# RoboticExplorationLab/TortoiseSat.jl

Measured on AMD Instinct MI355X. Metric: AL-iLQR trajectory solves/sec (1000 knots), higher is better.
Workload: dtype f64

## Files before the change

### tortoisesat.jl_amd/csrc/tsat_device.hpp

```cpp
#pragma once
#include <stdint.h>
#include "../../include/tortoise_hip.h"

#ifdef TSAT_EMU
#include <cmath>
namespace tsat_emu { int lane(); void sync(); void* lds(); double* xch(); }
#define TSAT_DEV inline
#define TSAT_PHASE inline
#define TSAT_FWD inline
#define TSAT_GLOBAL
#define TSAT_CONSTMEM
#define TSAT_LANE() (tsat_emu::lane())
#define TSAT_SYNC() (tsat_emu::sync())
#define TSAT_SYNC_LDS() (tsat_emu::sync())
#define TSAT_SCHED_FENCE() ((void)0)
#define TSAT_WAIT_LDS() ((void)0)
#define TSAT_NO_UNROLL
#define TSAT_ATOMIC_ADD(ptr, v) __atomic_fetch_add((ptr), (v), __ATOMIC_RELAXED)
#define TSAT_ATOMIC_LOAD(ptr) __atomic_load_n((ptr), __ATOMIC_RELAXED)
#define TSAT_UNIFORM_INT(x) (x)
#else
#define TSAT_DEV __device__ __forceinline__
#define TSAT_PHASE __device__ __noinline__
#if defined(TSAT_DENSE)
#define TSAT_FWD __device__ __noinline__
#else
#define TSAT_FWD __device__ __forceinline__
#endif
#if defined(__HIP_DEVICE_COMPILE__) && __HIP_DEVICE_COMPILE__
#define TSAT_GLOBAL __attribute__((address_space(1)))
#define TSAT_CONSTMEM __attribute__((address_space(4)))
#else
#define TSAT_GLOBAL
#define TSAT_CONSTMEM
#endif
#define TSAT_LANE() ((int)threadIdx.x)
#define TSAT_SYNC() __syncthreads()
#define TSAT_SYNC_LDS()                                       \
  do {                                                        \
    __builtin_amdgcn_fence(__ATOMIC_RELEASE, "wavefront");    \
    __builtin_amdgcn_wave_barrier();                          \
    __builtin_amdgcn_fence(__ATOMIC_ACQUIRE, "wavefront");    \
  } while (0)
#define TSAT_SCHED_FENCE() __builtin_amdgcn_sched_barrier(0)
#define TSAT_WAIT_LDS() __builtin_amdgcn_s_waitcnt(0xC07F)
#define TSAT_NO_UNROLL _Pragma("unroll 1")
#define TSAT_ATOMIC_ADD(ptr, v) atomicAdd((ptr), (v))
#define TSAT_ATOMIC_LOAD(ptr) __hip_atomic_load((ptr), __ATOMIC_RELAXED, __HIP_MEMORY_SCOPE_AGENT)
#define TSAT_UNIFORM_INT(x) __builtin_amdgcn_readfirstlane((int)(x))
#endif

#if !defined(TSAT_EMU)
#pragma clang fp contract(on)
#endif

namespace tsat {

#ifdef TSAT_F32
typedef float cfg_real;
#else
typedef double cfg_real;
#endif
typedef double acc_t;
constexpr int RPU = 16 / (int)sizeof(cfg_real);
#ifdef TSAT_JAC32
typedef float jac_t;
#else
typedef cfg_real jac_t;
#endif
constexpr int RPUJ = 16 / (int)sizeof(jac_t);

#if defined(TSAT_F32) && !defined(TSAT_OCC)
#define TSAT_OCC 2
#endif

constexpr int WAVE = 64;
#if defined(TSAT_F32) && TSAT_OCC == 4
constexpr int CK = 16;
#else
constexpr int CK = 32;
#endif
constexpr int PSTRIDE = 64;
constexpr int NSTORE = 12;
constexpr int N_FEW = 4;
enum { P_X0 = 0, P_XF = 7, P_QD = 14, P_QFD = 21, P_RD = 28, P_ULO = 31, P_UHI = 34, P_J = 37, P_JI = 46,
       P_TAU0 = 55, P_DTAU = 56, P_DT = 57,
       P_TAU0L = 61, P_DTAUL = 62 };
constexpr int FS = 7;
template <int ES> struct PkRec {
  static constexpr int FSR = ES ? 6 : FS;
  static constexpr int QQ = 54;
  static constexpr int LX = ES ? 60 : 70, LU = ES ? 66 : 77, LUU = ES ? 69 : 80;
  static constexpr int RECS = ES ? 72 : 84;
  static constexpr int SLOT = (64 / 16) * RECS + RPUJ;
};
struct TvRec {
  static constexpr int FSR = FS, LX = 70, LU = 77, LUU = 80, QQ = 83, RECS = 89;
};
constexpr int TV_CHB = 52;
template <int ES> struct BwdCfg {
  static constexpr int NH = ES ? 6 : 7;
  static constexpr int RECS = PkRec<ES>::RECS;
#if defined(TSAT_F32)
  static constexpr int CHB = (TSAT_OCC == 2) ? (ES ? 63 : 54) : (TSAT_OCC == 3) ? (ES ? 39 : 34) : (ES ? 27 : 23);
#elif defined(TSAT_JAC32) && defined(TSAT_DENSE)
  static constexpr int CHB = ES ? 59 : 50;
#elif defined(TSAT_JAC32)
  static constexpr int CHB = 64;
#elif defined(TSAT_DENSE)
  static constexpr int CHB = ES ? 29 : 25;
#else
  static constexpr int CHB = ES ? 64 : 55;
#endif
};
constexpr int KDW = 24, XUW = 10, LMW = 6, BSW = 9;
template <typename real> constexpr size_t pad16(size_t n) { return (n + (16 / sizeof(real)) - 1) / (16 / sizeof(real)) * (16 / sizeof(real)); }
template <typename real> constexpr size_t xu_stride(int NS) { return pad16<real>((size_t)NS * XUW); }
template <typename real> constexpr size_t kd_stride(int NS) { return (size_t)(NS - 1) * KDW; }
template <typename real> constexpr size_t lam_stride(int NS) { return pad16<real>((size_t)(NS - 1) * LMW); }
template <typename real> constexpr size_t u0_stride(int NS) { return (size_t)(NS - 1) * 3; }

template <typename real>
struct KArgs {
  int T, N, n_tab, max_ls;
  tsat_options opt;
  const real* P;
  const real* BT;
  const int* bidx;
  const int* nk;
  const real* U0;
  real* XU;
  real* KD;
  real* LAM;
  real* CAND;
  tsat_stats* stats;
  double* trace;
  int trace_rows;
  real* JW;
  int pk_few = 0;
  int suspend_at = 0;
  int* live = nullptr;
  int* susp_n = nullptr;
  int* susp_ids = nullptr;
  void* susp_state = nullptr;
};

constexpr int TSAT_JW_REALS_PER_4 = 16 * (4 * 84 + 4);

template <typename real>
struct TPtrs {
  TSAT_GLOBAL real* XU;
  TSAT_GLOBAL real* KD;
  TSAT_GLOBAL real* LAM;
  TSAT_GLOBAL real* CAND;
  const TSAT_GLOBAL real* bt;
  TSAT_GLOBAL real* XU0;
  int cur;
};
TSAT_DEV int cand_slab(int cur, int c) { return (c < cur) ? c : c + 1; }
template <typename real>
TSAT_DEV TSAT_GLOBAL real* slab_ptr(const TPtrs<real>& p, int N, int id) {
  return (id == 0) ? p.XU0 : p.CAND + (size_t)(id - 1) * (size_t)N * XUW;
}

constexpr int L_RED = 0;
constexpr int L_TR = L_RED + 64;
constexpr int TR_HJI = PSTRIDE, TR_HH = PSTRIDE + 9, TR_US = PSTRIDE + 10;
// ... 1374 lines not shown
          l = p.LAM[(size_t)k * LMW + 3 + m] + mu * clo;
          l = l > 0 ? l : (real)0; l = l < dmax ? l : dmax;
          p.LAM[(size_t)k * LMW + 3 + m] = l;
        }
      }
    } else {
      for (int i = 0; i < 7; ++i)
        if ((term_mask >> i) & 1) c = fmax_(c, fabs_(p.XU[(size_t)k * XUW + i] - tr.xf[i]));
    }
  }
  return wave_max(c, lds + L_RED);
}

template <typename real>
TSAT_PHASE real adopt_and_gradient(TPtrs<real> p, int N, int jw) {
  real* lds = lds_base<real>();
  const int lane = TSAT_LANE();
  const TSAT_GLOBAL real* Cg = p.CAND + (size_t)(jw >= 0 ? jw : 0) * (size_t)N * XUW;
  real g = 0;
  for (int k = lane; k < N; k += WAVE) {
    real r[10];
    const TSAT_GLOBAL real* src = (jw >= 0) ? (Cg + (size_t)k * XUW) : (p.XU + (size_t)k * XUW);
    for (int i = 0; i < 10; ++i) r[i] = src[i];
    if (jw >= 0)
      for (int i = 0; i < 10; ++i) p.XU[(size_t)k * XUW + i] = r[i];
    if (k < N - 1) {
      real m = 0;
      for (int c = 0; c < 3; ++c) m = fmax_(m, fabs_(p.KD[(size_t)k * KDW + 21 + c]) / (fabs_(r[7 + c]) + (real)1));
      g += m;
    }
  }
  g = wave_sum(g, lds + L_RED);
  return g / (real)(N - 1);
}

template <typename real>
TSAT_PHASE real todorov_gradient(const TSAT_GLOBAL real* XUs, const TSAT_GLOBAL real* KDg, int N) {
  real* lds = lds_base<real>();
  const int lane = TSAT_LANE();
  real g = 0;
  for (int k = lane; k < N - 1; k += WAVE) {
    real m = 0;
    for (int c = 0; c < 3; ++c) m = fmax_(m, fabs_(KDg[(size_t)k * KDW + 21 + c]) / (fabs_(XUs[(size_t)k * XUW + 7 + c]) + (real)1));
    g += m;
  }
  g = wave_sum(g, lds + L_RED);
  return g / (real)(N - 1);
}

template <typename real>
struct Resume {
  acc_t Jprev;
  real mu, rho, drho, grad, nu[7];
  int outer, it, djz, inner_iters, ls_trials, n_backward, n_forward, bp_restarts, fp_fails, trow;
  int cur, pad;
};

template <typename real, int INTEG, int DIAGJ, int ES>
TSAT_DEV int solve_trajectory(const KArgs<real>& a, int traj, const Resume<real>* rs = nullptr) {
  real* lds = lds_base<real>();
  const int lane = TSAT_LANE();
  const tsat_options& o = a.opt;
  const int NS = a.N, n_tab = a.n_tab;
  const int N = a.nk ? a.nk[traj] : a.N;
  TPtrs<real> p;
  p.XU = (TSAT_GLOBAL real*)(a.XU + (size_t)traj * xu_stride<real>(NS));
  p.KD = (TSAT_GLOBAL real*)(a.KD + (size_t)traj * kd_stride<real>(NS));
  p.LAM = (TSAT_GLOBAL real*)(a.LAM + (size_t)traj * lam_stride<real>(NS));
  p.CAND = (TSAT_GLOBAL real*)(a.CAND + (size_t)traj * a.max_ls * xu_stride<real>(NS));
  p.bt = (const TSAT_GLOBAL real*)(a.BT + (size_t)a.bidx[traj] * n_tab * 4);
  p.XU0 = p.XU; p.cur = 0;
#define TSAT_ADOPT(slot) do { p.cur = cand_slab(p.cur, (slot)); p.XU = slab_ptr<real>(p, N, p.cur); } while (0)
  stage_traj<real>((const TSAT_GLOBAL real*)(a.P + (size_t)traj * PSTRIDE), (real)o.u_scale);

  const real* U0g = a.U0 + (size_t)traj * u0_stride<real>(NS);
  double* trace = a.trace ? a.trace + (size_t)traj * a.trace_rows * 8 : nullptr;
  int trow = 0;
  real mu = (real)o.penalty_init;
  const real max_state = (real)o.max_state;
  const int tmask = o.terminal_mask;
  int status = TSAT_MAX_OUTER, outer_iters = 0, inner_iters = 0, ls_trials = 0, n_backward = 0, n_forward = 0,
      bp_restarts = 0, fp_fails = 0;
  real grad = 0;
  int last_jw = 0;
  unsigned long long pc_fwd = 0, pc_par = 0;
  bool start_ok = true;

  if (rs) {
    trow = rs->trow; mu = rs->mu; grad = rs->grad;
    p.cur = rs->cur; p.XU = slab_ptr<real>(p, N, p.cur);
    inner_iters = rs->inner_iters; ls_trials = rs->ls_trials; n_backward = rs->n_backward; n_forward = rs->n_forward;
    bp_restarts = rs->bp_restarts; fp_fails = rs->fp_fails;
    if (lane < 7) lds[L_NU + lane] = rs->nu[lane];
    TSAT_SYNC();
  } else {
    for (int k = lane; k < N; k += WAVE) {
      for (int i = 0; i < 7; ++i) p.XU[(size_t)k * XUW + i] = 0;
      for (int c = 0; c < 3; ++c) p.XU[(size_t)k * XUW + 7 + c] = (k < N - 1) ? U0g[(size_t)k * 3 + c] : (real)0;
      if (k < N - 1)
        for (int c = 0; c < 6; ++c) p.LAM[(size_t)k * LMW + c] = 0;
    }
    TSAT_SYNC();
    forward_sweep<real, INTEG, DIAGJ, ES>(p, N, n_tab, 0, 1, 0);
    n_forward++;
    TSAT_SYNC();
    const FwdOut<real> f0 = candidate_costs<real>(p, N, 0, 1, mu, tmask, max_state);
    const acc_t J0 = wave_bcast(f0.J, 0, red64());
    const int ok0 = wave_first<real>(!f0.ok, lds + L_RED) > 0;
    TSAT_SYNC();
    TSAT_ADOPT(0);
    start_ok = ok0 && (J0 - J0 == 0);
  }
  if (!start_ok) {
    status = TSAT_DIVERGED;
  } else {
    bool resumed = rs != nullptr;
    for (int outer = rs ? rs->outer : 1; outer <= o.max_outer; ++outer) {
      acc_t Jprev;
      real rho = (real)o.reg_init, drho = 0;
      int djz = 0, it0 = 1;
      if (resumed) {
        Jprev = rs->Jprev; rho = rs->rho; drho = rs->drho; djz = rs->djz; it0 = rs->it;
        resumed = false;
      } else {
        Jprev = nominal_cost<real>(p, N, mu, tmask, 1);
      }
      bool regfail = false;
      for (int it = it0; it <= o.max_inner; ++it) {
#ifdef TSAT_PACKED
        if (rs && a.suspend_at && a.live) {
          int* seen = reinterpret_cast<int*>(lds + L_RED);
          TSAT_SYNC_LDS();
          if (lane == 0) seen[0] = TSAT_ATOMIC_LOAD(a.live);
          TSAT_SYNC_LDS();
          const int live_now = seen[0];
          TSAT_SYNC_LDS();
          if (live_now <= a.suspend_at) {
            if (lane == 0) {
              const int pos = TSAT_ATOMIC_ADD(a.susp_n, 1);
              a.susp_ids[pos] = traj;
              Resume<real>& r = reinterpret_cast<Resume<real>*>(a.susp_state)[pos];
              r.Jprev = Jprev; r.mu = mu; r.rho = rho; r.drho = drho; r.grad = grad;
              for (int i = 0; i < 7; ++i) r.nu[i] = lds[L_NU + i];
              r.outer = outer; r.it = it; r.djz = djz; r.inner_iters = inner_iters; r.ls_trials = ls_trials;
              r.n_backward = n_backward; r.n_forward = n_forward; r.bp_restarts = bp_restarts; r.fp_fails = fp_fails; r.trow = trow;
              r.cur = p.cur; r.pad = 0;
            }
            TSAT_SYNC();
            return 1;
          }
        }
#endif
        BwdOut<real> bw;
        for (;;) {
          n_backward++;
          bw = backward_sweep<real, INTEG, DIAGJ, ES>(p, N, n_tab, mu, rho, tmask);
          if (bw.pd_ok) break;
          bp_restarts++;
          drho = (drho * (real)o.reg_scale > (real)o.reg_scale) ? drho * (real)o.reg_scale : (real)o.reg_scale;
          rho = (rho * drho > (real)o.reg_min) ? rho * drho : (real)o.reg_min;
          if (rho > (real)o.reg_max) { regfail = true; break; }
        }
        if (regfail) break;
        const acc_t dV1 = bw.dV1, dV2 = bw.dV2;
        const real rho_used = rho;
        {
          const real inv = (real)1 / (real)o.reg_scale;
          drho = (drho / (real)o.reg_scale < inv) ? drho / (real)o.reg_scale : inv;
          const real r = rho * drho;
          rho = (r > (real)o.reg_min) ? r : (real)0;
        }
        TSAT_SYNC();
        const unsigned long long t_f0 = tick_();
        const int n_slots = (o.max_linesearch < a.max_ls) ? o.max_linesearch : a.max_ls;
        int jw = WAVE, slot = 0;
        acc_t Jw = 0;
        unsigned long long t_cost = 0;
        int n_store = (last_jw >= N_FEW - 1 || n_slots < N_FEW) ? n_slots : N_FEW;
        for (int shift = 0; shift < o.max_linesearch && jw == WAVE; shift += n_store, n_store = n_slots) {
          const int n_here = (o.max_linesearch - shift < n_store) ? o.max_linesearch - shift : n_store;
          forward_sweep<real, INTEG, DIAGJ, ES>(p, N, n_tab, 1, n_here, shift);
          n_forward++;
          TSAT_SYNC();
          const unsigned long long t_c0 = tick_();
          for (int c0 = 0; c0 < n_here && jw == WAVE; c0 += CG) {
            const int nc = (n_here - c0 < CG) ? n_here - c0 : CG;
            const FwdOut<real> fw = candidate_costs<real>(p, N, c0, nc, mu, tmask, max_state);
            const int ci = shift + c0 + lane;
            acc_t alpha = 1;
            for (int j = 0; j < ci && j < TSAT_MAX_LINESEARCH; ++j) alpha *= (acc_t)0.5;
            const acc_t Jc = fw.J;
            const acc_t expected = -alpha * (dV1 + alpha * dV2);
            const acc_t z = (expected > 0) ? (Jprev - Jc) / expected : (acc_t)-1;
            const bool acc = (lane < nc) && fw.ok && ((z > (acc_t)o.ls_lower && z <= (acc_t)o.ls_upper) || Jc < Jprev);
            const int jl = wave_first<real>(acc, lds + L_RED);
            if (jl < WAVE) {
              jw = shift + c0 + jl;
              slot = c0 + jl;
              Jw = wave_bcast(Jc, jl, red64());
            }
          }
          t_cost += tick_() - t_c0;
        }
        const unsigned long long t_f1 = tick_();
        pc_fwd += (t_f1 - t_f0) - t_cost;
        pc_par += t_cost;
        acc_t J;
        TSAT_SYNC();
        last_jw = (jw < WAVE) ? jw : o.max_linesearch;
        if (jw < WAVE) {
          J = Jw;
          ls_trials += jw + 1;
          TSAT_ADOPT(slot);
          grad = todorov_gradient<real>(p.XU, p.KD, N);
        } else {
          J = Jprev;
          ls_trials += o.max_linesearch;
          fp_fails++;
          drho = (drho * (real)o.reg_scale > (real)o.reg_scale) ? drho * (real)o.reg_scale : (real)o.reg_scale;
          rho = (rho * drho > (real)o.reg_min) ? rho * drho : (real)o.reg_min;
          rho += (real)o.reg_fp;
          grad = todorov_gradient<real>(p.XU, p.KD, N);
        }
        TSAT_SYNC();
        pc_par += tick_() - t_f1;
        acc_t dJ = J - Jprev;
        dJ = dJ < 0 ? -dJ : dJ;
        if (trace && lane == 0 && trow < a.trace_rows) {
          double* r = trace + 8 * trow;
          r[0] = outer; r[1] = it; r[2] = (double)Jprev; r[3] = (double)J; r[4] = (jw < WAVE) ? jw : -1;
          r[5] = (double)rho_used; r[6] = (double)dV1; r[7] = (double)dV2;
#if defined(TSAT_PROFILE) && !defined(TSAT_EMU)
          r[7] = (double)wall_clock64();
#endif
        }
        trow++;
        Jprev = J;
        djz = (dJ == 0) ? djz + 1 : 0;
        inner_iters++;
        if (0 < dJ && dJ < (acc_t)o.cost_tol) break;
        if (grad < (real)o.grad_tol) break;
        if (djz > o.dj_counter_limit) break;
      }
      outer_iters = outer;
      const real cmax = violation_and_duals<real>(p, N, mu, tmask, 0, (real)o.dual_max);
      if (regfail) { status = TSAT_REG_FAIL; break; }
      if (cmax < (real)o.constraint_tol) { status = TSAT_CONVERGED; break; }
      if (outer == o.max_outer) break;
      (void)violation_and_duals<real>(p, N, mu, tmask, 1, (real)o.dual_max);
      if (lane < 7 && ((tmask >> lane) & 1)) {
        const real dmax = (real)o.dual_max;
        real v = lds[L_NU + lane] + mu * (p.XU[(size_t)(N - 1) * XUW + lane] - lds[L_TR + P_XF + lane]);
        v = v > -dmax ? v : -dmax; v = v < dmax ? v : dmax;
        lds[L_NU + lane] = v;
      }
      mu = (mu * (real)o.penalty_scale < (real)o.penalty_max) ? mu * (real)o.penalty_scale : (real)o.penalty_max;
      TSAT_SYNC();
    }
  }
  TSAT_SYNC();
  if (p.cur != 0) {
    for (int k = lane; k < N; k += WAVE)
      for (int i = 0; i < XUW; ++i) p.XU0[(size_t)k * XUW + i] = p.XU[(size_t)k * XUW + i];
    p.XU = p.XU0; p.cur = 0;
    TSAT_SYNC();
  }
  const real cmax = violation_and_duals<real>(p, N, mu, tmask, 0, (real)o.dual_max);
  const acc_t cost = nominal_cost<real>(p, N, mu, tmask, 0);
  const acc_t cost_al = nominal_cost<real>(p, N, mu, tmask, 1);
  if (lane == 0) {
    tsat_stats& st = a.stats[traj];
    st.status = status; st.outer_iters = outer_iters; st.inner_iters = inner_iters; st.ls_trials = ls_trials;
    st.n_backward = n_backward; st.n_forward = n_forward; st.bp_restarts = bp_restarts; st.fp_fails = fp_fails;
    st.cost = (double)cost; st.cost_al = (double)cost_al; st.c_max = (double)cmax; st.grad = (double)grad;
#ifdef TSAT_PROFILE
    if (trace && a.trace_rows > 0) {
      trace[0] = (double)pc_fwd; trace[1] = (double)lds[L_PC + 1]; trace[2] = (double)lds[L_PC + 2];
      trace[3] = (double)pc_par; trace[4] = (double)inner_iters; trace[5] = (double)n_backward;
    }
#else
    (void)pc_fwd; (void)pc_par;
#endif
  }
  return 0;
}

constexpr int P_QATT = 58;

template <typename real>
struct TvArgs {
  int T, N, n_tab, lin_sq, min_steps;
  real us, w_tol, ang_tol;
// ... 558 lines not shown
```

### tortoisesat.jl_amd/csrc/tsat_kernels.hip

```cpp
#include <hip/hip_runtime.h>
#include <algorithm>
#include <atomic>
#include <cmath>
#include <thread>
#include <dlfcn.h>
#include <rccl/rccl.h>
#include <cstdio>
#include <cstdlib>
#include <cstring>
#include <string>
#include <vector>
#include "tsat_host_pack.hpp"

using namespace tsat;

hipError_t tsat_launch_solve_dense(const KArgs<double>& a, int rk4, int inertia_class, int error_state, hipStream_t stream);
hipError_t tsat_launch_solve_packed(const KArgs<double>& a, int rk4, int inertia_class, int error_state, hipStream_t stream);
hipError_t tsat_launch_solve_packed8(const KArgs<double>& a, int rk4, int inertia_class, int error_state, hipStream_t stream);
hipError_t tsat_launch_solve_packed8w(const KArgs<double>& a, int rk4, int inertia_class, int error_state, hipStream_t stream);
hipError_t tsat_launch_solve_packed16w(const KArgs<double>& a, int rk4, int inertia_class, int error_state, hipStream_t stream);
hipError_t tsat_launch_solve_packed4w(const KArgs<double>& a, int rk4, int inertia_class, int error_state, hipStream_t stream);
hipError_t tsat_launch_solve_dense_mixed(const KArgs<double>& a, int rk4, int inertia_class, int error_state, hipStream_t stream);
hipError_t tsat_launch_solve_packed_mixed(const KArgs<double>& a, int rk4, int inertia_class, int error_state, hipStream_t stream);
hipError_t tsat_launch_solve_packed_mixed8(const KArgs<double>& a, int rk4, int inertia_class, int error_state, hipStream_t stream);
hipError_t tsat_launch_solve_packed_mixed8w(const KArgs<double>& a, int rk4, int inertia_class, int error_state, hipStream_t stream);
hipError_t tsat_launch_solve_packed_mixed16w(const KArgs<double>& a, int rk4, int inertia_class, int error_state, hipStream_t stream);
hipError_t tsat_launch_solve_packed_mixed4w(const KArgs<double>& a, int rk4, int inertia_class, int error_state, hipStream_t stream);

template <typename real, int INTEG, int DIAGJ, int ES>
__global__ __launch_bounds__(64) void tsat_solve_kernel(KArgs<real> a) {
  const int traj = blockIdx.x;
  if (traj >= a.T) return;
  solve_trajectory<real, INTEG, DIAGJ, ES>(a, traj);
}

template <typename real, int DIAGJ>
__global__ __launch_bounds__(64) void tsat_tvlqr_kernel(TvArgs<real> a) {
  const int traj = blockIdx.x;
  if (traj >= a.T) return;
  tvlqr_trajectory<real, DIAGJ>(a, traj);
}

template <typename real, int DIAGJ>
__global__ __launch_bounds__(64) void tsat_mpc_advance_kernel(MpcArgs<real> a) {
  const int traj = blockIdx.x;
  if (traj >= a.T) return;
  mpc_advance_trajectory<real, DIAGJ>(a, traj);
}

template <typename real>
__global__ __launch_bounds__(64) void tsat_btable_kernel(BtArgs<real> a) {
  const int traj = blockIdx.x;
  if (traj >= a.T) return;
  btable_trajectory<real>(a, traj);
}

template <typename real>
__global__ __launch_bounds__(64) void tsat_horizon_kernel(HzArgs<real> a) {
  const int traj = blockIdx.x;
  if (traj >= a.T) return;
  horizon_trajectory<real>(a, traj);
}

__global__ __launch_bounds__(256) void tsat_pack_tables_kernel(int64_t n, int rows, int n_tab, const double* B, double* BT) {
  const int64_t e = (int64_t)blockIdx.x * blockDim.x + threadIdx.x;
  if (e >= n) return;
  const int64_t t = e / n_tab;
  const int r = (int)(e - t * n_tab);
  const double* src = B + ((size_t)t * rows + r) * 3;
  double* dst = BT + (size_t)e * 4;
  dst[0] = src[0]; dst[1] = src[1]; dst[2] = src[2]; dst[3] = 0.0;
}
template <typename real>
__global__ __launch_bounds__(256) void tsat_export_kernel(int64_t n_rec, int N, const int* nk, const real* XU,
                                                          const real* KD, double* X, double* U, double* K) {
  const int64_t e = (int64_t)blockIdx.x * blockDim.x + threadIdx.x;
  if (e < n_rec) export_record<real>(e, N, nk, XU, KD, X, U, K);
}

struct tsat_handle {
  int dev = -1;
  hipStream_t stream = nullptr;
  hipEvent_t ev0 = nullptr, ev1 = nullptr;
  std::string err;
  int64_t T = 0, n_btab = 0;
  int N = 0, n_tab = 0, max_ls = 0, trace_rows = 0;
  bool uploaded = false, solved = false;
  int inertia_class = 0;
  double *P = nullptr, *BT = nullptr, *U0 = nullptr, *XU = nullptr, *KD = nullptr, *LAM = nullptr, *CAND = nullptr;
  int* bidx = nullptr;
  int* nk = nullptr;
  bool ragged = false;
  tsat_stats* stats = nullptr;
  double* trace = nullptr;
  int64_t bytes = 0;
  int endgame = -1;
  int variant = 0;
  std::vector<double> hx0, hxf, htau0, hdtau, hdt, hJ;
  int64_t bt_T = 0;
  int bt_rows = 0;
  int64_t bt_gen = 0;
  enum { WS_TV_NZ, WS_TV_KD, WS_TV_XS, WS_TV_NID, WS_TV_ST, WS_TV_P, WS_TVB_P, WS_TVB_BT, WS_TVB_XUR, WS_TVB_BI, WS_TVB_NK,
         WS_HZ_B, WS_HZ_DT, WS_HZ_CUT, WS_HZ_C, WS_HZ_I, WS_BT_COEF, WS_BT_KEP, WS_BT_T0, WS_BT_TF, WS_BT_POS, WS_BT_B,
         WS_JW, WS_MPC_HX, WS_MPC_HU,
         WS_DL_X, WS_DL_U, WS_DL_K, WS_AG_X, WS_AG_U, WS_AG_ST, WS_AG_XA, WS_AG_UA, WS_AG_STA,
         WS_AG_CHK, WS_MPC_TALLY, WS_ENDGAME, WS_COUNT };
  void* ws[WS_COUNT] = {};
  size_t ws_bytes[WS_COUNT] = {};
  void* comm = nullptr;
  int comm_rank = 0, comm_world = 1;
  int64_t comm_T = -1; int comm_N = -1;
  int64_t mpc_tally_T = 0;
};

namespace {

int fail(tsat_handle* h, int code, const std::string& msg) {
  if (h) h->err = msg;
  return code;
}
#define TSAT_HIP(h, call)                                                                      \
  do {                                                                                         \
    hipError_t e_ = (call);                                                                    \
    if (e_ != hipSuccess)                                                                      \
      return fail((h), -10, std::string(#call) + ": " + hipGetErrorString(e_));                \
  } while (0)

void release(tsat_handle* h) {
  void* ptrs[] = {h->P, h->BT, h->U0, h->XU, h->KD, h->LAM, h->CAND, h->bidx, h->nk, h->stats, h->trace};
  for (void* p : ptrs)
    if (p) (void)hipFree(p);
  h->P = h->BT = h->U0 = h->XU = h->KD = h->LAM = h->CAND = nullptr;
  h->bidx = nullptr; h->nk = nullptr; h->ragged = false; h->stats = nullptr; h->trace = nullptr;
  h->T = 0; h->bytes = 0; h->uploaded = h->solved = false;
}

void* ws_get(tsat_handle* h, int slot, size_t bytes) {
  if (bytes == 0) bytes = 16;
  if (h->ws[slot] && h->ws_bytes[slot] >= bytes) return h->ws[slot];
  if (h->ws[slot]) { (void)hipFree(h->ws[slot]); h->ws[slot] = nullptr; h->ws_bytes[slot] = 0; }
  void* p = nullptr;
  if (hipMalloc(&p, bytes) != hipSuccess) return nullptr;
  h->ws[slot] = p;
  h->ws_bytes[slot] = bytes;
  return p;
}
void ws_release(tsat_handle* h) {
  for (int i = 0; i < tsat_handle::WS_COUNT; ++i)
    if (h->ws[i]) { (void)hipFree(h->ws[i]); h->ws[i] = nullptr; h->ws_bytes[i] = 0; }
}

template <typename Tp>
int dev_alloc(tsat_handle* h, Tp** p, size_t n) {
  const size_t b = n * sizeof(Tp);
  TSAT_HIP(h, hipMalloc(reinterpret_cast<void**>(p), b ? b : 16));
  h->bytes += (int64_t)b;
  return 0;
}

}

extern "C" {

int tsat_version(void) { return 300; }

void tsat_default_options(tsat_options* o) {
  std::memset(o, 0, sizeof(*o));
  o->integrator = 3; o->precision = 64;
  o->max_outer = 20; o->max_inner = 50;
  o->max_linesearch = 20; o->dj_counter_limit = 10;
  o->cost_tol = 1e-4; o->grad_tol = 1e-5; o->constraint_tol = 1e-3;
  o->penalty_init = 1.0; o->penalty_scale = 10.0; o->penalty_max = 1e8; o->dual_max = 1e8;
  o->reg_init = 0.0; o->reg_scale = 1.6; o->reg_min = 1e-8; o->reg_max = 1e8; o->reg_fp = 10.0;
  o->ls_lower = 1e-8; o->ls_upper = 10.0; o->max_state = 1e8;
  o->u_scale = 1e-2;
  o->terminal_mask = 0x7f; o->error_state = 0;
}

int tsat_create(tsat_handle** out, int device_id) {
  if (!out) return -1;
  *out = nullptr;
  int n = 0;
  if (hipGetDeviceCount(&n) != hipSuccess || n <= 0) return -2;
  if (device_id < 0 || device_id >= n) return -3;
  hipDeviceProp_t prop;
  if (hipGetDeviceProperties(&prop, device_id) != hipSuccess) return -4;
  if (std::strncmp(prop.gcnArchName, "gfx950", 6) != 0) return -5;
  if (hipSetDevice(device_id) != hipSuccess) return -6;
  tsat_handle* h = new tsat_handle();
  h->dev = device_id;
  if (hipStreamCreateWithFlags(&h->stream, hipStreamNonBlocking) != hipSuccess ||
      hipEventCreate(&h->ev0) != hipSuccess || hipEventCreate(&h->ev1) != hipSuccess) {
    delete h;
    return -7;
  }
  *out = h;
  return 0;
}

int tsat_destroy(tsat_handle* h) {
  if (!h) return -1;
  (void)hipSetDevice(h->dev);
  (void)tsat_comm_destroy(h);
  release(h);
  ws_release(h);
  if (h->ev0) (void)hipEventDestroy(h->ev0);
  if (h->ev1) (void)hipEventDestroy(h->ev1);
  if (h->stream) (void)hipStreamDestroy(h->stream);
  delete h;
  return 0;
}

const char* tsat_last_error(const tsat_handle* h) { return h ? h->err.c_str() : "null handle"; }

int64_t tsat_batch_bytes(const tsat_handle* h) { return h ? h->bytes : 0; }

int64_t tsat_workspace_bytes(const tsat_handle* h) {
  int64_t b = 0;
  if (h)
    for (int i = 0; i < tsat_handle::WS_COUNT; ++i) b += (int64_t)h->ws_bytes[i];
  return b;
}

int tsat_workspace_trim(tsat_handle* h, int32_t what) {
  if (!h) return -1;
  if (what != 0 && what != 1) return fail(h, -1, "what must be 0 (staging buffers of downloads and gathers) or 1 (every workspace)");
  TSAT_HIP(h, hipSetDevice(h->dev));
  TSAT_HIP(h, hipStreamSynchronize(h->stream));
  for (int i = 0; i < tsat_handle::WS_COUNT; ++i) {
    const bool staging = i >= tsat_handle::WS_DL_X && i <= tsat_handle::WS_AG_STA;
    if (!h->ws[i] || !(what == 1 || staging)) continue;
    (void)hipFree(h->ws[i]);
    h->ws[i] = nullptr; h->ws_bytes[i] = 0;
    if (i == tsat_handle::WS_BT_B) { h->bt_T = 0; h->bt_rows = 0; h->bt_gen++; }
  }
  return 0;
}

int64_t tsat_btable_generation(const tsat_handle* h) { return h ? h->bt_gen : 0; }

int tsat_batch_reserve(tsat_handle* h, int64_t T, int32_t n_knots, int32_t n_tab, int64_t n_btab,
                       int32_t max_linesearch) {
  if (!h) return -1;
  if (T < 1 || n_knots < 2 || n_tab < 1 || n_btab < 1) return fail(h, -1, "bad batch dimensions");
  if (max_linesearch < 1 || max_linesearch > TSAT_MAX_LINESEARCH) return fail(h, -1, "max_linesearch must be in [1,32]");
  TSAT_HIP(h, hipSetDevice(h->dev));
  if (h->T == T && h->N == n_knots && h->n_tab == n_tab && h->n_btab == n_btab && h->max_ls == max_linesearch)
    return 0;
  const int trows = h->trace_rows;
  release(h);
  const size_t N = (size_t)n_knots, Tn = (size_t)T;
  int rc = 0;
  rc |= dev_alloc(h, &h->P, Tn * PSTRIDE);
  rc |= dev_alloc(h, &h->BT, (size_t)n_btab * n_tab * 4);
  rc |= dev_alloc(h, &h->bidx, Tn);
  rc |= dev_alloc(h, &h->nk, Tn);
  rc |= dev_alloc(h, &h->U0, Tn * (N - 1) * 3);
  rc |= dev_alloc(h, &h->XU, Tn * N * XUW);
  rc |= dev_alloc(h, &h->KD, Tn * (N - 1) * KDW);
  rc |= dev_alloc(h, &h->LAM, Tn * (N - 1) * LMW);
  const int slots = max_linesearch < NSTORE ? max_linesearch : NSTORE;
  rc |= dev_alloc(h, &h->CAND, Tn * (size_t)slots * N * XUW);
  rc |= dev_alloc(h, &h->stats, Tn);
  if (trows > 0) rc |= dev_alloc(h, &h->trace, Tn * (size_t)trows * 8);
  if (rc) { release(h); return -10; }
  h->T = T; h->N = n_knots; h->n_tab = n_tab; h->n_btab = n_btab; h->max_ls = max_linesearch;
  h->trace_rows = trows;
  return 0;
}

int tsat_batch_trace(tsat_handle* h, int32_t rows) {
  if (!h || rows < 0) return -1;
  TSAT_HIP(h, hipSetDevice(h->dev));
  if (h->trace) { (void)hipFree(h->trace); h->trace = nullptr; }
  h->trace_rows = rows;
  if (rows > 0 && h->T > 0) {
    if (dev_alloc(h, &h->trace, (size_t)h->T * rows * 8)) return -10;
  }
  return 0;
}

int tsat_batch_upload(tsat_handle* h, const double* x0, const double* xf, const double* Btab,
                      const int32_t* btab_idx, const double* tau0, const double* dtau, const double* dt,
                      const double* Jmat, const double* Qd, const double* Qfd, const double* Rd,
                      const double* ulo, const double* uhi, const double* U0) {
  if (!h) return -1;
  if (h->T < 1) return fail(h, -1, "tsat_batch_reserve has not been called");
  if (!x0 || !xf || !tau0 || !dtau || !dt || !Jmat || !Qd || !Qfd || !Rd || !ulo || !uhi || !U0)
    return fail(h, -1, "null input array");
  if (!Btab && (h->bt_T != h->T || h->n_btab != h->T || h->n_tab > h->bt_rows))
    return fail(h, -1, "Btab is NULL but the field tables left by the last tsat_btable_batch do not cover this batch "
                       "(need one table per trajectory, n_btab = T, and n_tab <= its 2 n_half rows)");
  if (!btab_idx && h->n_btab != h->T) return fail(h, -1, "btab_idx is NULL but n_btab != T");
  TSAT_HIP(h, hipSetDevice(h->dev));
  const int64_t T = h->T;
  std::vector<int> bi((size_t)T);
  for (int64_t t = 0; t < T; ++t) {
    const int64_t v = btab_idx ? btab_idx[t] : t;
    if (v < 0 || v >= h->n_btab) return fail(h, -1, "btab_idx out of range");
    bi[(size_t)t] = (int)v;
  }
  const std::string bad = check_inputs(T, x0, xf, tau0, dtau, dt, Jmat, Qd, Qfd, Rd, ulo, uhi);
  if (!bad.empty()) return fail(h, -1, bad);
  h->inertia_class = inertia_class(T, Jmat);
  std::vector<double> P((size_t)T * PSTRIDE);
  pack_params<double>(T, x0, xf, tau0, dtau, dt, Jmat, Qd, Qfd, Rd, ulo, uhi, P.data());
  TSAT_HIP(h, hipMemcpy(h->P, P.data(), P.size() * sizeof(double), hipMemcpyHostToDevice));
  if (Btab) {
    std::vector<double> BT((size_t)h->n_btab * h->n_tab * 4);
    pack_btab<double>(h->n_btab, h->n_tab, Btab, BT.data());
    TSAT_HIP(h, hipMemcpy(h->BT, BT.data(), BT.size() * sizeof(double), hipMemcpyHostToDevice));
  } else {
    const int64_t n = T * (int64_t)h->n_tab;
    const double* B = (const double*)ws_get(h, tsat_handle::WS_BT_B, (size_t)h->bt_T * h->bt_rows * 3 * 8);
    if (!B) return fail(h, -10, "resident field tables are gone");
    hipLaunchKernelGGL(tsat_pack_tables_kernel, dim3((unsigned)((n + 255) / 256)), dim3(256), 0, h->stream, n, h->bt_rows, h->n_tab, B, h->BT);
    TSAT_HIP(h, hipGetLastError());
    TSAT_HIP(h, hipStreamSynchronize(h->stream));
  }
  TSAT_HIP(h, hipMemcpy(h->bidx, bi.data(), bi.size() * sizeof(int), hipMemcpyHostToDevice));
  TSAT_HIP(h, hipMemcpy(h->U0, U0, (size_t)T * (h->N - 1) * 3 * sizeof(double), hipMemcpyHostToDevice));
  h->hx0.assign(x0, x0 + 7 * T); h->hxf.assign(xf, xf + 7 * T); h->htau0.assign(tau0, tau0 + T);
  h->hdtau.assign(dtau, dtau + T); h->hdt.assign(dt, dt + T); h->hJ.assign(Jmat, Jmat + 9 * T);
  h->uploaded = true;
  h->solved = false;
  h->ragged = false;
  return 0;
}

int tsat_batch_knots(tsat_handle* h, const int32_t* n_knots) {
  if (!h) return -1;
  if (!h->uploaded) return fail(h, -1, "tsat_batch_upload has not been called");
  if (!n_knots) { h->ragged = false; return 0; }
  for (int64_t t = 0; t < h->T; ++t)
    if (n_knots[t] < 2 || n_knots[t] > h->N) return fail(h, -1, "n_knots[t] must be in [2, N]");
  TSAT_HIP(h, hipSetDevice(h->dev));
  TSAT_HIP(h, hipMemcpy(h->nk, n_knots, (size_t)h->T * sizeof(int), hipMemcpyHostToDevice));
  h->ragged = true;
  h->solved = false;
  return 0;
}

namespace {
using solve_kern_t = void (*)(KArgs<double>);
solve_kern_t solve_variant(const tsat_handle* h, const tsat_options* o) {
  static const solve_kern_t variants[2][3][2] = {
      {{tsat_solve_kernel<double, 3, 0, 0>, tsat_solve_kernel<double, 3, 0, 1>},
       {tsat_solve_kernel<double, 3, 1, 0>, tsat_solve_kernel<double, 3, 1, 1>},
       {tsat_solve_kernel<double, 3, 2, 0>, tsat_solve_kernel<double, 3, 2, 1>}},
      {{tsat_solve_kernel<double, 4, 0, 0>, tsat_solve_kernel<double, 4, 0, 1>},
       {tsat_solve_kernel<double, 4, 1, 0>, tsat_solve_kernel<double, 4, 1, 1>},
       {tsat_solve_kernel<double, 4, 2, 0>, tsat_solve_kernel<double, 4, 2, 1>}}};
  return variants[o->integrator == 4 ? 1 : 0][h->inertia_class][o->error_state ? 1 : 0];
}

constexpr int64_t TSAT_WIDE_MAX_T = 1024;
constexpr int64_t TSAT_PACKED_MIN_T = 2048, TSAT_PACKED4W_MAX_T = 4096;
constexpr int64_t TSAT_PACKED8W_MAX_T = 8192;
constexpr int64_t TSAT_PACKED16W_MIN_T = 16384, TSAT_LONG_BUDGET = 100;
int selected_build(const tsat_handle* h, int precision, int64_t budget) {
  if (h->variant >= 3) return h->variant;
  if (h->variant == 0 && h->T >= TSAT_PACKED16W_MIN_T) return budget >= TSAT_LONG_BUDGET ? 4 : 6;
  if (h->variant == 0 && h->T > TSAT_PACKED8W_MAX_T) return 4;
  if (h->variant == 0 && h->T > TSAT_PACKED4W_MAX_T) return 5;
  if (h->variant == 0 && h->T >= TSAT_PACKED_MIN_T) return 7;
  if (precision == 32) return 2;
  return (h->variant == 2 || (h->variant != 1 && h->T > TSAT_WIDE_MAX_T)) ? 2 : 1;
}
hipError_t launch_solve(const tsat_handle* h, const tsat_options* o, const KArgs<double>& a) {
  const int build = selected_build(h, o->precision, (int64_t)o->max_outer * o->max_inner), rk4 = o->integrator == 4;
  if (o->precision == 32) {
    if (build == 7) return tsat_launch_solve_packed_mixed4w(a, rk4, h->inertia_class, o->error_state, h->stream);
    if (build == 6) return tsat_launch_solve_packed_mixed16w(a, rk4, h->inertia_class, o->error_state, h->stream);
    if (build == 5) return tsat_launch_solve_packed_mixed8w(a, rk4, h->inertia_class, o->error_state, h->stream);
    if (build == 4) return tsat_launch_solve_packed_mixed8(a, rk4, h->inertia_class, o->error_state, h->stream);
    if (build == 3) return tsat_launch_solve_packed_mixed(a, rk4, h->inertia_class, o->error_state, h->stream);
    return tsat_launch_solve_dense_mixed(a, rk4, h->inertia_class, o->error_state, h->stream);
  }
  if (build == 7) return tsat_launch_solve_packed4w(a, rk4, h->inertia_class, o->error_state, h->stream);
  if (build == 6) return tsat_launch_solve_packed16w(a, rk4, h->inertia_class, o->error_state, h->stream);
  if (build == 5) return tsat_launch_solve_packed8w(a, rk4, h->inertia_class, o->error_state, h->stream);
  if (build == 4) return tsat_launch_solve_packed8(a, rk4, h->inertia_class, o->error_state, h->stream);
  if (build == 3) return tsat_launch_solve_packed(a, rk4, h->inertia_class, o->error_state, h->stream);
  if (build == 2) return tsat_launch_solve_dense(a, rk4, h->inertia_class, o->error_state, h->stream);
  hipLaunchKernelGGL(solve_variant(h, o), dim3((unsigned)h->T), dim3(64), 0, h->stream, a);
  return hipGetLastError();
}

void* packed_workspace(tsat_handle* h) {
  return ws_get(h, tsat_handle::WS_JW, (size_t)((h->T + 3) / 4) * TSAT_JW_REALS_PER_4 * sizeof(double));
}

bool uses_packed_build(const tsat_handle* h, int precision) { return selected_build(h, precision, 0) >= 3; }

struct EndgameArgs { int suspend_at = 0; int *live = nullptr, *susp_n = nullptr, *susp_ids = nullptr; void* susp_state = nullptr; };
int endgame_threshold(const tsat_handle* h, const tsat_options* o) {
  int at = h->endgame;
  if (at < 0) at = ((int64_t)o->max_outer * o->max_inner >= 20) ? (int)std::min<int64_t>(2048, h->T / 8) : 0;
  return at <= 0 ? 0 : (int)std::min<int64_t>(at, h->T);
}
EndgameArgs endgame_args(tsat_handle* h, const tsat_options* o) {
  EndgameArgs a;
  const int at = endgame_threshold(h, o);
  if (at <= 0) return a;
  const size_t T = (size_t)h->T, ids_at = 16, st_at = (ids_at + T * sizeof(int) + 15) / 16 * 16;
  char* w = (char*)ws_get(h, tsat_handle::WS_ENDGAME, st_at + T * sizeof(Resume<double>));
  if (!w) return a;
  a.suspend_at = (int)std::min<int64_t>(at, h->T);
  a.live = (int*)w; a.susp_n = (int*)w + 1; a.susp_ids = (int*)(w + ids_at); a.susp_state = w + st_at;
  return a;
}

KArgs<double> solve_args(tsat_handle* h, const tsat_options* o) {
  KArgs<double> a;
  a.T = (int)h->T; a.N = h->N; a.n_tab = h->n_tab; a.max_ls = h->max_ls < NSTORE ? h->max_ls : NSTORE; a.opt = *o;
  a.P = h->P; a.BT = h->BT; a.bidx = h->bidx; a.nk = h->ragged ? h->nk : nullptr; a.U0 = h->U0;
  a.XU = h->XU; a.KD = h->KD; a.LAM = h->LAM; a.CAND = h->CAND;
  a.stats = h->stats; a.trace = h->trace; a.trace_rows = h->trace ? h->trace_rows : 0;
  a.JW = uses_packed_build(h, 64) ? (double*)packed_workspace(h) : nullptr;
  if (a.JW) {
    const EndgameArgs e = endgame_args(h, o);
    a.suspend_at = e.suspend_at; a.live = e.live; a.susp_n = e.susp_n; a.susp_ids = e.susp_ids; a.susp_state = e.susp_state;
  }
  return a;
}

}

int tsat_batch_run(tsat_handle* h, const tsat_options* o, float* kernel_ms) {
  if (!h || !o) return -1;
  if (!h->uploaded) return fail(h, -1, "tsat_batch_upload has not been called");
  const std::string why = check_options(*o, h->N, h->n_tab, h->max_ls);
  if (!why.empty()) return fail(h, -1, why);
  TSAT_HIP(h, hipSetDevice(h->dev));
  const KArgs<double> a = solve_args(h, o);
  if (!a.JW && uses_packed_build(h, 64))
    return fail(h, -10, "device allocation of the packed builds' Jacobian workspace failed");
  if (h->trace) TSAT_HIP(h, hipMemsetAsync(h->trace, 0, (size_t)h->T * h->trace_rows * 8 * sizeof(double), h->stream));
  TSAT_HIP(h, hipEventRecord(h->ev0, h->stream));
  TSAT_HIP(h, launch_solve(h, o, a));
  TSAT_HIP(h, hipEventRecord(h->ev1, h->stream));
  TSAT_HIP(h, hipStreamSynchronize(h->stream));
  if (kernel_ms) TSAT_HIP(h, hipEventElapsedTime(kernel_ms, h->ev0, h->ev1));
  h->solved = true;
  return 0;
}

int tsat_set_kernel_variant(tsat_handle* h, int32_t variant) {
  if (!h) return -1;
  if (!(variant >= 0 && variant <= 7))
    return fail(h, -1, "variant must be 0 (automatic), 1 (wide), 2 (dense), 3 (packed: 4 trajectories per wavefront), 4 (packed8), 5 (packed8w: 8, one wavefront per SIMD) or 6 (packed16w) or 7 (packed4w: 4, one wavefront per SIMD)");
  h->variant = variant;
  return 0;
}

int tsat_selected_build(tsat_handle* h, const tsat_options* o, int32_t* build, int32_t* endgame_at) {
  if (!h || !o) return -1;
  if (h->T <= 0) return fail(h, -1, "tsat_batch_reserve has not been called");
  const int b = selected_build(h, o->precision, (int64_t)o->max_outer * o->max_inner);
  if (build) *build = b;
  if (endgame_at) *endgame_at = b >= 3 ? endgame_threshold(h, o) : 0;
  return 0;
}

int tsat_set_endgame(tsat_handle* h, int32_t suspend_at) {
  if (!h) return -1;
  if (suspend_at < -1) return fail(h, -1, "suspend_at must be -1 (automatic), 0 (never) or the live count at which the packed builds park their trajectories");
  h->endgame = suspend_at;
  return 0;
}

int tsat_mpc_run(tsat_handle* h, const tsat_options* o, int32_t n_steps, int32_t plant_integrator, double* X_hist,
                 double* U_hist, tsat_stats* stats_last, float* solve_ms) {
  if (!h || !o) return -1;
  if (!h->uploaded) return fail(h, -1, "tsat_batch_upload has not been called");
  const std::string why = check_options(*o, h->N, h->n_tab, h->max_ls);
  if (!why.empty()) return fail(h, -1, why);
  if (n_steps < 1) return fail(h, -1, "n_steps must be >= 1");
  if (o->precision != 64) return fail(h, -1, "tsat_mpc_run runs the fp64 build only (precision must be 64)");
  if (plant_integrator != 3 && plant_integrator != 4) return fail(h, -1, "plant_integrator must be 3 (rk3) or 4 (rk4)");
  if (!X_hist || !U_hist) return fail(h, -1, "null array");
  TSAT_HIP(h, hipSetDevice(h->dev));
  const size_t T = (size_t)h->T, nX = T * ((size_t)n_steps + 1) * 7, nU = T * (size_t)n_steps * 3;
  double* dHX = (double*)ws_get(h, tsat_handle::WS_MPC_HX, nX * 8);
  double* dHU = (double*)ws_get(h, tsat_handle::WS_MPC_HU, nU * 8);
  long long* dTally = (long long*)ws_get(h, tsat_handle::WS_MPC_TALLY, T * 4 * sizeof(long long));
  if (!dHX || !dHU || !dTally) return fail(h, -10, "device allocation failed in tsat_mpc_run");
  TSAT_HIP(h, hipMemsetAsync(dTally, 0, T * 4 * sizeof(long long), h->stream));
  h->mpc_tally_T = (int64_t)T;
  const KArgs<double> a = solve_args(h, o);
  if (!a.JW && uses_packed_build(h, 64))
    return fail(h, -10, "device allocation of the packed builds' Jacobian workspace failed");
  MpcArgs<double> m;
  m.T = (int)h->T; m.N = h->N; m.n_tab = h->n_tab; m.plant_integ = plant_integrator; m.n_steps = n_steps; m.us = o->u_scale;
  m.P = h->P; m.BT = h->BT; m.bidx = h->bidx; m.nk = h->ragged ? h->nk : nullptr; m.XU = h->XU; m.U0 = h->U0;
  m.HX = dHX; m.HU = dHU; m.stats = h->stats; m.tally = dTally;
  auto adv = h->inertia_class == 2 ? tsat_mpc_advance_kernel<double, 2>
                                   : (h->inertia_class == 1 ? tsat_mpc_advance_kernel<double, 1> : tsat_mpc_advance_kernel<double, 0>);
// ... 460 lines not shown
```

### tortoisesat.jl_amd/csrc/tsat_packed.hpp

```cpp
#pragma once
#include "tsat_device.hpp"

namespace tsat {

#ifndef TSAT_PK_G
#define TSAT_PK_G 4
#endif
#ifndef TSAT_PK_CK
#define TSAT_PK_CK 4
#endif
#ifndef TSAT_PK_NBUF
#define TSAT_PK_NBUF 2
#endif
#ifndef TSAT_PK_STORE
#define TSAT_PK_STORE 6
#endif
#ifndef TSAT_PK_WAVES
#define TSAT_PK_WAVES 2
#endif
constexpr bool PK_ALONE = (TSAT_PK_WAVES == 1);
constexpr int PK_STORE = TSAT_PK_STORE;
constexpr int PK_FEW = 3;
constexpr int PK_G = TSAT_PK_G;
constexpr int PK_C = WAVE / PK_G;
constexpr int PK_CK = TSAT_PK_CK;
constexpr int PK_NBUF = TSAT_PK_NBUF;
static_assert(PK_G * PK_C == WAVE && (PK_C & (PK_C - 1)) == 0, "PK_G must be a power of two");
constexpr int PK_UKD = PK_CK * KDW / RPU, PK_ULM = PK_CK * LMW / RPU, PK_UXU = PK_CK * XUW / RPU;
static_assert((PK_CK * KDW) % RPU == 0 && (PK_CK * LMW) % RPU == 0 && (PK_CK * XUW) % RPU == 0, "chunks are whole 16-byte units");
constexpr int PK_SKD = (PK_UKD + 1) * RPU, PK_SLM = (PK_ULM + 1) * RPU, PK_SXU = (PK_UXU + 1) * RPU;
constexpr int PK_BROWS = PK_CK * 3 + 1;
constexpr int PK_SB = PK_BROWS * 4, PK_SGT = PK_SLM;
constexpr int PK_R_KD = 0, PK_R_LM = PK_R_KD + PK_G * PK_SKD, PK_R_XU = PK_R_LM + PK_G * PK_SLM, PK_R_B = PK_R_XU + PK_G * PK_SXU,
              PK_R_GT = PK_R_B + PK_G * PK_SB, PK_FB = PK_R_GT + PK_G * PK_SGT;
constexpr int PK_NI_KD = (PK_G * (PK_UKD + 1) + WAVE - 1) / WAVE, PK_NI_LM = (PK_G * (PK_ULM + 1) + WAVE - 1) / WAVE,
              PK_NI_XU = (PK_G * (PK_UXU + 1) + WAVE - 1) / WAVE, PK_NI_B = (PK_G * PK_BROWS * BROW_UNITS + WAVE - 1) / WAVE;
static_assert(L_FWD + PK_NBUF * PK_FB <= LDS_REALS, "packed forward buffers fit the wave's LDS block");

constexpr int PK_JCH = 16;
#ifndef TSAT_PK_RING
#define TSAT_PK_RING ((sizeof(jac_t) == 8) ? 4 : 8)
#endif
constexpr int PK_RING = TSAT_PK_RING;
constexpr int PK_CPB = 16;
constexpr int PK_BC = 16;
constexpr int PK_BG = WAVE / PK_BC;
static_assert(PK_G % PK_BG == 0 && PK_JCH == PK_BC, "Jacobian lanes: the 16 lanes of a trajectory linearise 16 knots");
constexpr int PK_RECS = 84;
constexpr int PK_GTRW = 88;
constexpr int PK_GT_NU = 76;
constexpr int PK_GXW = 64;
static_assert(PkRec<0>::RECS % RPUJ == 0 && PkRec<1>::RECS % RPUJ == 0 && PkRec<0>::RECS <= PK_RECS, "a record is a whole number of 16-byte units");
constexpr int L_GTR = L_UNION;
constexpr int L_GX = L_GTR + PK_BG * PK_GTRW;
constexpr int L_GREC = L_GX + PK_BG * PK_GXW;
constexpr int PK_SLOT = PK_BG * PK_RECS + RPUJ;
static_assert(L_GREC * (int)sizeof(cfg_real) + PK_RING * PK_SLOT * (int)sizeof(jac_t) <= LDS_REALS * (int)sizeof(cfg_real), "joint backward sweep fits the wave's LDS block");
constexpr int PK_JW_WAVE = PK_JCH * PK_SLOT;
TSAT_DEV jac_t* ring_base() { return reinterpret_cast<jac_t*>(lds_base<cfg_real>() + L_GREC); }
static_assert(PK_JW_WAVE <= TSAT_JW_REALS_PER_4, "host allocation of a.JW");
constexpr int sym_ut(int i, int j, int n) { return i * n - (i * (i - 1)) / 2 + (j - i); }
template <typename real> struct BwdIn { int N, need; real mu, rho; int cur, pad; };
template <typename real> struct BwdRes { acc_t dV1, dV2; int ok, pad; };
constexpr int L_BWT = L_WT;
static_assert(L_BWT % 2 == 0, "hand-over tables are 8-byte aligned");

template <typename real>
struct GState {
  acc_t Jprev, dV1, dV2, Jw;
  real mu, rho, drho, grad, rho_used, nu[7];
  int N, active, status, outer, it, inner_iters, ls_trials, n_backward, n_forward, bp_restarts, fp_fails, djz, trow, regfail,
      found, jw, slot, need_bwd, last_jw, cur;
};

template <typename real>
TSAT_DEV GState<real> gstate_bcast(const GState<real>& s, int src) {
  static_assert(sizeof(GState<real>) <= (L_UNION - L_ST) * sizeof(real), "state record fits the Riccati scratch");
  GState<real>* buf = reinterpret_cast<GState<real>*>(lds_base<real>() + L_ST);
  if (TSAT_LANE() == src) *buf = s;
  TSAT_SYNC_LDS();
  const GState<real> r = *buf;
  TSAT_SYNC_LDS();
  return r;
}

template <typename real>
TSAT_DEV TPtrs<real> group_ptrs(const KArgs<real>& a, int traj, int cur = 0, int N = 0) {
  const int NS = a.N;
  TPtrs<real> p;
  p.XU = (TSAT_GLOBAL real*)(a.XU + (size_t)traj * xu_stride<real>(NS));
  p.KD = (TSAT_GLOBAL real*)(a.KD + (size_t)traj * kd_stride<real>(NS));
  p.LAM = (TSAT_GLOBAL real*)(a.LAM + (size_t)traj * lam_stride<real>(NS));
  p.CAND = (TSAT_GLOBAL real*)(a.CAND + (size_t)traj * a.max_ls * xu_stride<real>(NS));
  p.bt = (const TSAT_GLOBAL real*)(a.BT + (size_t)a.bidx[traj] * a.n_tab * 4);
  p.XU0 = p.XU; p.cur = cur;
  if (cur) p.XU = slab_ptr<real>(p, N, cur);
  return p;
}

#ifdef TSAT_PK_FWD_INLINE
#define TSAT_PK_FWD TSAT_FWD
#else
#define TSAT_PK_FWD TSAT_PHASE
#endif
template <typename real, int INTEG, int DIAGJ, int ES>
// ... 751 lines not shown
```

Before: 13260.

## Raise non-packed candidate slots and drop adaptive few-candidate first line-search pass

Raises the candidate slab count for non-packed builds from 12 to 20 and removes the adaptive first pass that evaluated only a few candidates when the previous accepted step was early. Each line search now rolls out min(max_linesearch, slots) candidates in one forward sweep. Packed builds get their own smaller slab reservation, sized at allocation time from the selected build. The change trades fewer forward sweeps for extra rollouts when an early step would have been accepted, plus more memory traffic and a larger candidate buffer.

```diff
diff --git a/tortoisesat.jl_amd/csrc/tsat_device.hpp b/tortoisesat.jl_amd/csrc/tsat_device.hpp
--- a/tortoisesat.jl_amd/csrc/tsat_device.hpp
+++ b/tortoisesat.jl_amd/csrc/tsat_device.hpp
@@ -81,8 +81,8 @@
 constexpr int CK = 32;
 #endif
 constexpr int PSTRIDE = 64;
-constexpr int NSTORE = 12;
-constexpr int N_FEW = 4;
+constexpr int NSTORE = 20;
+constexpr int PK_SLOTS = 6;
 enum { P_X0 = 0, P_XF = 7, P_QD = 14, P_QFD = 21, P_RD = 28, P_ULO = 31, P_UHI = 34, P_J = 37, P_JI = 46,
        P_TAU0 = 55, P_DTAU = 56, P_DT = 57,
        P_TAU0L = 61, P_DTAUL = 62 };
@@ -1623,7 +1623,6 @@
   int status = TSAT_MAX_OUTER, outer_iters = 0, inner_iters = 0, ls_trials = 0, n_backward = 0, n_forward = 0,
       bp_restarts = 0, fp_fails = 0;
   real grad = 0;
-  int last_jw = 0;
   unsigned long long pc_fwd = 0, pc_par = 0;
   bool start_ok = true;
 
@@ -1713,12 +1712,11 @@
         }
         TSAT_SYNC();
         const unsigned long long t_f0 = tick_();
-        const int n_slots = (o.max_linesearch < a.max_ls) ? o.max_linesearch : a.max_ls;
+        const int n_store = (o.max_linesearch < a.max_ls) ? o.max_linesearch : a.max_ls;
         int jw = WAVE, slot = 0;
         acc_t Jw = 0;
         unsigned long long t_cost = 0;
-        int n_store = (last_jw >= N_FEW - 1 || n_slots < N_FEW) ? n_slots : N_FEW;
-        for (int shift = 0; shift < o.max_linesearch && jw == WAVE; shift += n_store, n_store = n_slots) {
+        for (int shift = 0; shift < o.max_linesearch && jw == WAVE; shift += n_store) {
           const int n_here = (o.max_linesearch - shift < n_store) ? o.max_linesearch - shift : n_store;
           forward_sweep<real, INTEG, DIAGJ, ES>(p, N, n_tab, 1, n_here, shift);
           n_forward++;
@@ -1748,7 +1746,6 @@
         pc_par += t_cost;
         acc_t J;
         TSAT_SYNC();
-        last_jw = (jw < WAVE) ? jw : o.max_linesearch;
         if (jw < WAVE) {
           J = Jw;
           ls_trials += jw + 1;
diff --git a/tortoisesat.jl_amd/csrc/tsat_kernels.hip b/tortoisesat.jl_amd/csrc/tsat_kernels.hip
--- a/tortoisesat.jl_amd/csrc/tsat_kernels.hip
+++ b/tortoisesat.jl_amd/csrc/tsat_kernels.hip
@@ -85,6 +85,7 @@
   std::string err;
   int64_t T = 0, n_btab = 0;
   int N = 0, n_tab = 0, max_ls = 0, trace_rows = 0;
+  int slots = 0;
   bool uploaded = false, solved = false;
   int inertia_class = 0;
   double *P = nullptr, *BT = nullptr, *U0 = nullptr, *XU = nullptr, *KD = nullptr, *LAM = nullptr, *CAND = nullptr;
@@ -132,8 +133,10 @@
     if (p) (void)hipFree(p);
   h->P = h->BT = h->U0 = h->XU = h->KD = h->LAM = h->CAND = nullptr;
   h->bidx = nullptr; h->nk = nullptr; h->ragged = false; h->stats = nullptr; h->trace = nullptr;
-  h->T = 0; h->bytes = 0; h->uploaded = h->solved = false;
-}
+  h->T = 0; h->slots = 0; h->bytes = 0; h->uploaded = h->solved = false;
+}
+
+int selected_build(int variant, int64_t T, int precision, int64_t budget);
 
 void* ws_get(tsat_handle* h, int slot, size_t bytes) {
   if (bytes == 0) bytes = 16;
@@ -259,12 +262,13 @@
   rc |= dev_alloc(h, &h->XU, Tn * N * XUW);
   rc |= dev_alloc(h, &h->KD, Tn * (N - 1) * KDW);
   rc |= dev_alloc(h, &h->LAM, Tn * (N - 1) * LMW);
-  const int slots = max_linesearch < NSTORE ? max_linesearch : NSTORE;
+  const int cap = selected_build(h->variant, T, 64, 0) >= 3 ? PK_SLOTS : NSTORE;
+  const int slots = max_linesearch < cap ? max_linesearch : cap;
   rc |= dev_alloc(h, &h->CAND, Tn * (size_t)slots * N * XUW);
   rc |= dev_alloc(h, &h->stats, Tn);
   if (trows > 0) rc |= dev_alloc(h, &h->trace, Tn * (size_t)trows * 8);
   if (rc) { release(h); return -10; }
-  h->T = T; h->N = n_knots; h->n_tab = n_tab; h->n_btab = n_btab; h->max_ls = max_linesearch;
+  h->T = T; h->N = n_knots; h->n_tab = n_tab; h->n_btab = n_btab; h->max_ls = max_linesearch; h->slots = slots;
   h->trace_rows = trows;
   return 0;
 }
@@ -358,15 +362,16 @@
 constexpr int64_t TSAT_PACKED_MIN_T = 2048, TSAT_PACKED4W_MAX_T = 4096;
 constexpr int64_t TSAT_PACKED8W_MAX_T = 8192;
 constexpr int64_t TSAT_PACKED16W_MIN_T = 16384, TSAT_LONG_BUDGET = 100;
-int selected_build(const tsat_handle* h, int precision, int64_t budget) {
-  if (h->variant >= 3) return h->variant;
-  if (h->variant == 0 && h->T >= TSAT_PACKED16W_MIN_T) return budget >= TSAT_LONG_BUDGET ? 4 : 6;
-  if (h->variant == 0 && h->T > TSAT_PACKED8W_MAX_T) return 4;
-  if (h->variant == 0 && h->T > TSAT_PACKED4W_MAX_T) return 5;
-  if (h->variant == 0 && h->T >= TSAT_PACKED_MIN_T) return 7;
+int selected_build(int variant, int64_t T, int precision, int64_t budget) {
+  if (variant >= 3) return variant;
+  if (variant == 0 && T >= TSAT_PACKED16W_MIN_T) return budget >= TSAT_LONG_BUDGET ? 4 : 6;
+  if (variant == 0 && T > TSAT_PACKED8W_MAX_T) return 4;
+  if (variant == 0 && T > TSAT_PACKED4W_MAX_T) return 5;
+  if (variant == 0 && T >= TSAT_PACKED_MIN_T) return 7;
   if (precision == 32) return 2;
-  return (h->variant == 2 || (h->variant != 1 && h->T > TSAT_WIDE_MAX_T)) ? 2 : 1;
-}
+  return (variant == 2 || (variant != 1 && T > TSAT_WIDE_MAX_T)) ? 2 : 1;
+}
+int selected_build(const tsat_handle* h, int precision, int64_t budget) { return selected_build(h->variant, h->T, precision, budget); }
 hipError_t launch_solve(const tsat_handle* h, const tsat_options* o, const KArgs<double>& a) {
   const int build = selected_build(h, o->precision, (int64_t)o->max_outer * o->max_inner), rk4 = o->integrator == 4;
   if (o->precision == 32) {
@@ -413,7 +418,7 @@
 
 KArgs<double> solve_args(tsat_handle* h, const tsat_options* o) {
   KArgs<double> a;
-  a.T = (int)h->T; a.N = h->N; a.n_tab = h->n_tab; a.max_ls = h->max_ls < NSTORE ? h->max_ls : NSTORE; a.opt = *o;
+  a.T = (int)h->T; a.N = h->N; a.n_tab = h->n_tab; a.max_ls = h->slots; a.opt = *o;
   a.P = h->P; a.BT = h->BT; a.bidx = h->bidx; a.nk = h->ragged ? h->nk : nullptr; a.U0 = h->U0;
   a.XU = h->XU; a.KD = h->KD; a.LAM = h->LAM; a.CAND = h->CAND;
   a.stats = h->stats; a.trace = h->trace; a.trace_rows = h->trace ? h->trace_rows : 0;
diff --git a/tortoisesat.jl_amd/csrc/tsat_packed.hpp b/tortoisesat.jl_amd/csrc/tsat_packed.hpp
--- a/tortoisesat.jl_amd/csrc/tsat_packed.hpp
+++ b/tortoisesat.jl_amd/csrc/tsat_packed.hpp
@@ -21,6 +21,7 @@
 constexpr bool PK_ALONE = (TSAT_PK_WAVES == 1);
 constexpr int PK_STORE = TSAT_PK_STORE;
 constexpr int PK_FEW = 3;
+static_assert(PK_STORE <= PK_SLOTS, "tsat_batch_reserve reserves PK_SLOTS candidate slabs per trajectory for the packed builds");
 constexpr int PK_G = TSAT_PK_G;
 constexpr int PK_C = WAVE / PK_G;
 constexpr int PK_CK = TSAT_PK_CK;
```

After: 13410, median of 6. 1.01x the previous value.
